# HuajianUP/Photo-SLAM

Hardware: AMD Instinct MI355X
Metric: train iters/s (render + L1/SSIM loss + backward + Adam), 2M Gaussians @1080p (higher is better)
Workload: dtype f32; 1 GPU; C3: Replica room0 @1080p shape; gaussians=2000000, width=1920, height=1080, sh_degree=3, parallelism=single GPU, raster_only=False, densify_interval=0, cull_empty_tiles=False, binning=depth-first, sh_adam_fused_into_backward=True, sh_adam_lazy_window=32, scene_index_order=random, geometry_adam_fused_into_backward=True, gaussians_after=2000000

## Files before the change

photo-slam_amd/csrc/preprocess.hip:

```cpp
#include "state.h"
#include "wave64.h"
#include "kernels.h"
#include "shrows.h"

namespace gsr {


__device__ __forceinline__ int f2i(float f)
{
	if (f != f) return 0;
	if (f >= 2147483648.0f) return 2147483647;
	if (f <= -2147483648.0f) return (-2147483647 - 1);
	return (int)f;
}

__device__ __forceinline__ float ndc2pix(float v, int S) { return (float)(((v + 1.0) * S - 1.0) * 0.5); }

#ifndef GSR_FWD_STAGE_ROWS
#define GSR_FWD_STAGE_ROWS STAGE_ROWS
#endif
constexpr int FWD_ROWS = GSR_FWD_STAGE_ROWS;

template <bool AA>
__global__ void __launch_bounds__(PRE_THREADS)
preprocess_fwd_kernel(const PreprocessParams p, GeometryState g)
{
	__shared__ float4 s_rows[PRE_THREADS / 64][FWD_ROWS][ROW_F4_PAD];
	__shared__ uint32_t s_list[PRE_THREADS / 64][64];
	__shared__ uint32_t s_lag[PRE_THREADS / 64][64];

	const int idx = (int)(blockIdx.x * blockDim.x + threadIdx.x);
	for (int t = idx; t < p.tiles; t += (int)(gridDim.x * blockDim.x)) p.ranges[t] = make_uint2(0u, 0u);
	for (int t = idx; t < LONG_LISTS * LONG_COUNT_STRIDE; t += (int)(gridDim.x * blockDim.x)) g.long_counts[t] = 0u;
	const int w = wave_id();
	const size_t wave_first = (size_t)(blockIdx.x * blockDim.x) + (size_t)w * 64;
	const bool in_range = idx < p.P;
	const int row_step = (p.lazy.row_step != nullptr && in_range) ? p.lazy.row_step[idx] : 0;
	uint32_t my_tiles = 0;
	int radius_i = 0;
	uint32_t depth_key = DEPTH_KEY_CULLED;
	float px = 0.f, py = 0.f, pz = 0.f;
	float pix = 0.f, piy = 0.f, conx = 0.f, cony = 0.f, conz = 0.f;
	uint32_t rect_lo = 0, rect_hi = 0;
	float aa_h = 1.0f;

	if (in_range) {
		do {
			px = p.means3D[3 * idx];
			py = p.means3D[3 * idx + 1];
			pz = p.means3D[3 * idx + 2];
			const float* V = p.view;
			const float* Pm = p.proj;
			const float vz = V[2] * px + V[6] * py + V[10] * pz + V[14];
			if (vz <= 0.2f) break;
			const float hx = Pm[0] * px + Pm[4] * py + Pm[8] * pz + Pm[12];
			const float hy = Pm[1] * px + Pm[5] * py + Pm[9] * pz + Pm[13];
			const float hw = Pm[3] * px + Pm[7] * py + Pm[11] * pz + Pm[15];
			const float p_w = 1.0f / (hw + 0.0000001f);
			const float projx = hx * p_w, projy = hy * p_w;

			float c3[6];
			if (p.cov3D_precomp != nullptr) {
#pragma unroll
				for (int i = 0; i < 6; i++) c3[i] = p.cov3D_precomp[6 * (size_t)idx + i];
			} else {
				compute_cov3D(p.scales, p.rotations, (size_t)idx, p.scale_modifier, p.raw_params, c3);
			}

			float tx = V[0] * px + V[4] * py + V[8] * pz + V[12];
			float ty = V[1] * px + V[5] * py + V[9] * pz + V[13];
			const float tz = vz;
			const float limx = 1.3f * p.tan_fovx, limy = 1.3f * p.tan_fovy;
			const float txtz = tx / tz, tytz = ty / tz;
			tx = fminf(limx, fmaxf(-limx, txtz)) * tz;
// ... 24 lines not shown
			const float lambda2 = mid - sqrtf(fmaxf(0.1f, mid * mid - det));
			const float my_radius = ceilf(3.f * sqrtf(fmaxf(lambda1, lambda2)));
			pix = ndc2pix(projx, p.W);
			piy = ndc2pix(projy, p.H);
			const int mr = f2i(my_radius);
			const int rminx = min(p.grid_x, max(0, f2i((pix - mr) / TILE)));
			const int rminy = min(p.grid_y, max(0, f2i((piy - mr) / TILE)));
			const int rmaxx = min(p.grid_x, max(0, f2i((pix + mr + TILE - 1) / TILE)));
			const int rmaxy = min(p.grid_y, max(0, f2i((piy + mr + TILE - 1) / TILE)));
			const uint32_t tiles = (uint32_t)(rmaxy - rminy) * (uint32_t)(rmaxx - rminx);
			if (tiles == 0) break;
			if (p.cov3D_precomp == nullptr && (p.raw_params & GSR_STORE_COV3D)) {
#pragma unroll
				for (int i = 0; i < 6; i++) g.cov3D[6 * (size_t)idx + i] = c3[i];
			}
			depth_key = __float_as_uint(vz);
			radius_i = mr;
			my_tiles = tiles;
			rect_lo = (uint32_t)rminx | ((uint32_t)rminy << 16);
			rect_hi = (uint32_t)rmaxx | ((uint32_t)rmaxy << 16);
		} while (0);
	}
	const bool vis = my_tiles != 0;

	float cr = 0.f, cg = 0.f, cb = 0.f;
	uint8_t clamp_bits = 0;
	if (p.colors_precomp == nullptr) {
		const int ncoef = (p.D + 1) * (p.D + 1);
		const bool rows_ok = (p.M * 3 == ROW_F4 * 4) && ((reinterpret_cast<uintptr_t>(p.shs) & 15) == 0);
		float rgb[3] = {0.f, 0.f, 0.f};
		auto direction = [&]() {
			const float dx = px - p.campos[0], dy = py - p.campos[1], dz = pz - p.campos[2];
			const float len = sqrtf(dx * dx + dy * dy + dz * dz);
			return sh_dir(dx / len, dy / len, dz / len);
		};
		if (rows_ok) {
			const unsigned long long vmask = wave_ballot(vis);
			const int nvis = __popcll(vmask);
			const int rank = __popcll(vmask & lanemask_lt());
			int lag = 0;
			if (p.lazy.row_step != nullptr && vis) {
				lag = p.lazy.step - 1 - row_step;
				lag = lag < 0 ? 0 : (lag >= p.lazy.window ? p.lazy.window - 1 : lag);
			}
			const bool lagging = wave_ballot(lag > 0) != 0;
			if (vis) {
				s_list[w][rank] = (uint32_t)lane_id();
				s_lag[w][rank] = (uint32_t)lag;
			}
			wave_fence();
			const int nf4 = lagging ? ROW_F4 : (3 * ncoef + 3) >> 2;
			for (int r0 = 0; r0 < nvis; r0 += FWD_ROWS) {
				const int count = (nvis - r0) < FWD_ROWS ? (nvis - r0) : FWD_ROWS;
				wave_load_listed_rows(reinterpret_cast<const float4*>(p.shs), wave_first, nf4, r0, count, s_rows[w], s_list[w]);
				if (lagging) {
					if (p.forward_only) wave_lazy_peek_listed(p.lazy, wave_first, r0, count, s_rows[w], s_list[w], s_lag[w]);
					else wave_lazy_catch_up_listed(p.lazy, wave_first, r0, count, s_rows[w], s_list[w], s_lag[w]);
				}
				if (vis && rank >= r0 && rank < r0 + count) sh_row_to_rgb(s_rows[w][rank - r0], ncoef, direction(), rgb);
				wave_fence();
			}
			if (lag > 0 && !p.forward_only) p.lazy.row_step[idx] = p.lazy.step - 1;
		} else if (vis) {
			const float* sh = p.shs + (size_t)idx * p.M * 3;
			const ShDir d = direction();
#pragma unroll
			for (int k = 0; k < 16; k++) {
				if (k < ncoef) {
#pragma unroll
					for (int ch = 0; ch < 3; ch++) {
						const float t = sh_basis(k, d) * sh[3 * k + ch];
						rgb[ch] = (k == 0) ? t : rgb[ch] + t;
					}
				}
			}
		}
		if (vis) {
			cr = rgb[0] + 0.5f;
			cg = rgb[1] + 0.5f;
			cb = rgb[2] + 0.5f;
			clamp_bits = (uint8_t)((cr < 0 ? 1 : 0) | (cg < 0 ? 2 : 0) | (cb < 0 ? 4 : 0));
			cr = fmaxf(cr, 0.0f);
			cg = fmaxf(cg, 0.0f);
			cb = fmaxf(cb, 0.0f);
		}
	} else if (vis) {
		cr = p.colors_precomp[3 * (size_t)idx];
		cg = p.colors_precomp[3 * (size_t)idx + 1];
		cb = p.colors_precomp[3 * (size_t)idx + 2];
	}

	if (in_range) {
		if (vis) {
			g.rec[3 * (size_t)idx + 0] = make_float4(pix, piy, conx, cony);
			float opac = p.opacities[idx];
			if (p.raw_params & GSR_RAW_OPACITY) opac = 1.0f / (1.0f + expf(-opac));
			if constexpr (AA) opac = opac * aa_h;
			g.rec[3 * (size_t)idx + 1] = make_float4(conz, opac, cr, cg);
			g.rec[3 * (size_t)idx + 2] = make_float4(cb, __uint_as_float(rect_lo), __uint_as_float(rect_hi), 0.f);
			if (!p.forward_only) g.clamped[idx] = clamp_bits;
			reinterpret_cast<uint2*>(g.rect)[idx] = make_uint2(rect_lo, rect_hi);
		}
		g.depth_key[idx] = depth_key;
		g.tiles_touched[idx] = my_tiles;
		g.radii[idx] = radius_i;
		if (p.radii_out) p.radii_out[idx] = radius_i;
	}
// ... 33 lines not shown
```

photo-slam_amd/csrc/preprocess_bwd.hip:

```cpp
#include "state.h"
#include "wave64.h"
#include <stdlib.h>
#include "kernels.h"
#include "shrows.h"
#include "partials.h"

namespace gsr {


constexpr int PRB_THREADS = 128;
constexpr int SHB_THREADS = 64;

template <int N>
__device__ __forceinline__ void geom_adam_row(const GeomAdamTensor& t, size_t idx, const float (&g)[N])
{
#pragma unroll
	for (int k = 0; k < N; k++) {
		const size_t i = (size_t)N * idx + k;
		const float m = t.s.b1 * t.exp_avg[i] + t.s.omb1 * g[k];
		const float v = t.s.b2 * t.exp_avg_sq[i] + t.s.omb2 * g[k] * g[k];
		t.exp_avg[i] = m;
		t.exp_avg_sq[i] = v;
		t.param[i] -= t.s.step_size * adam_ratio(m, v, t.s.inv_sqrt_bc2, t.s.eps);
	}
}
__device__ __forceinline__ void geom_adam_row4(const GeomAdamTensor& t, size_t idx, const float4& g4)
{
	float4 pv = reinterpret_cast<const float4*>(t.param)[idx];
	float4 mv = reinterpret_cast<const float4*>(t.exp_avg)[idx];
	float4 vv = reinterpret_cast<const float4*>(t.exp_avg_sq)[idx];
	float* pp = &pv.x; float* mp = &mv.x; float* vp = &vv.x;
	const float g[4] = {g4.x, g4.y, g4.z, g4.w};
#pragma unroll
	for (int k = 0; k < 4; k++) {
		mp[k] = t.s.b1 * mp[k] + t.s.omb1 * g[k];
		vp[k] = t.s.b2 * vp[k] + t.s.omb2 * g[k] * g[k];
		pp[k] -= t.s.step_size * adam_ratio(mp[k], vp[k], t.s.inv_sqrt_bc2, t.s.eps);
	}
	reinterpret_cast<float4*>(t.param)[idx] = pv;
	reinterpret_cast<float4*>(t.exp_avg)[idx] = mv;
	reinterpret_cast<float4*>(t.exp_avg_sq)[idx] = vv;
}

template <int DEG, int MODE, bool POSE = false>
#ifndef GSR_SHB_WAVES_LO
#define GSR_SHB_WAVES_LO 6
#endif
__global__ void __launch_bounds__(SHB_THREADS) GSR_WAVES_PER_EU(GSR_SHB_WAVES_LO, 8)
sh_bwd_rows_kernel(const PreprocessBwdParams p)
{
	__shared__ float4 s_rows[SHB_THREADS / 64][STAGE_ROWS][ROW_F4_PAD];
	__shared__ uint32_t s_list[SHB_THREADS / 64][STAGE_ROWS];
	__shared__ float s_aux[SHB_THREADS / 64][MODE == 2 ? STAGE_ROWS : 1][AUX_PITCH];
	const int idx = (int)(blockIdx.x * blockDim.x + threadIdx.x);
	const int w = wave_id(), l = lane_id();
	const size_t wave_first = (size_t)(blockIdx.x * blockDim.x) + (size_t)w * 64;
	if (p.touched_clear)
		for (uint32_t o = 16u * (uint32_t)idx; o < p.touched_clear_bytes; o += 16u * (uint32_t)(gridDim.x * blockDim.x))
			*reinterpret_cast<uint4*>(p.touched_clear + o) = make_uint4(0u, 0u, 0u, 0u);
	const bool in_range = idx < p.P;
	const bool vis = in_range && (p.radii[idx] > 0);
	constexpr int ncoef = (DEG + 1) * (DEG + 1);
	constexpr bool FACTORED = MODE == 1;
	float dRGB[3] = {0.f, 0.f, 0.f};
	float ddx[3] = {0.f, 0.f, 0.f}, ddy[3] = {0.f, 0.f, 0.f}, ddz[3] = {0.f, 0.f, 0.f};
	float ox = 0.f, oy = 0.f, oz = 1.f;
	if (vis) {
		ox = p.means3D[3 * (size_t)idx] - p.campos[0];
		oy = p.means3D[3 * (size_t)idx + 1] - p.campos[1];
		oz = p.means3D[3 * (size_t)idx + 2] - p.campos[2];
		if (FACTORED) {
			dRGB[0] = p.dL_dcolor_view[3 * (size_t)idx + 0];
			dRGB[1] = p.dL_dcolor_view[3 * (size_t)idx + 1];
			dRGB[2] = p.dL_dcolor_view[3 * (size_t)idx + 2];
		} else {
			const uint8_t cl = p.clamped[idx];
			dRGB[0] = p.dL_dcolor[3 * (size_t)idx + 0] * ((cl & 1) ? 0.f : 1.f);
			dRGB[1] = p.dL_dcolor[3 * (size_t)idx + 1] * ((cl & 2) ? 0.f : 1.f);
			dRGB[2] = p.dL_dcolor[3 * (size_t)idx + 2] * ((cl & 4) ? 0.f : 1.f);
		}
	}
	{
		{
			const int nf4 = MODE == 2 ? ROW_F4 : (3 * ncoef + 3) >> 2;
#pragma unroll 1
			for (int h = 0; h < 64 / STAGE_ROWS; h++) {
				const size_t half_first = wave_first + (size_t)(h * STAGE_ROWS);
				const long long left = (long long)p.P - (long long)half_first;
				if (left <= 0) break;
				const bool mine = (l / STAGE_ROWS) == h;
				const unsigned long long m = wave_ballot(vis && mine);
				if (vis && mine) s_list[w][__popcll(m & lanemask_lt())] = (uint32_t)(l % STAGE_ROWS);
				wave_fence();
				wave_load_listed_rows<true>(reinterpret_cast<const float4*>(p.shs), half_first, nf4, 0, __popcll(m), s_rows[w], s_list[w]);
				if (mine && in_range) {
					float4* row = s_rows[w][l % STAGE_ROWS];
					if (vis) {
						float ux = ox, uy = oy, uz = oz;
						GSR_OPAQUE_F32(ux);
						GSR_OPAQUE_F32(uy);
						GSR_OPAQUE_F32(uz);
						const float len = sqrtf(ux * ux + uy * uy + uz * uz);
						const ShDir d = sh_dir(ux / len, uy / len, uz / len);
						sh_row_backward<MODE == 0>(row, ncoef, d, dRGB, ddx, ddy, ddz);
						if (MODE == 2) {
							float* ax = s_aux[w][l % STAGE_ROWS];
#pragma unroll
							for (int k = 0; k < 16; k++) ax[k] = k < ncoef ? sh_basis(k, d) : 0.f;
							ax[16] = dRGB[0];
							ax[17] = dRGB[1];
							ax[18] = dRGB[2];
						}
					} else if (MODE == 0) {
#pragma unroll
						for (int i = 0; i < ROW_F4; i++) row[i] = make_float4(0.f, 0.f, 0.f, 0.f);
					}
				}
				if (MODE == 0) {
					wave_store_rows(reinterpret_cast<float4*>(p.dL_dsh), half_first, (int)(left > STAGE_ROWS ? STAGE_ROWS : left), s_rows[w]);
				} else if (MODE == 2) {
					const RowAdam ra = {p.adam_param, p.adam_exp_avg, p.adam_exp_avg_sq, p.adam};
					const uint32_t lit = (uint32_t)(m >> (h * STAGE_ROWS));
					const uint32_t rows = p.adam_skip_culled ? lit : 0xFFFFFFFFu;
					wave_adam_rows_rank1(ra, half_first, (int)(left > STAGE_ROWS ? STAGE_ROWS : left), s_rows[w], s_aux[w], rows, lit);
				} else {
					wave_fence();
				}
			}
		}
	}
	if (MODE == 2 && vis && p.lazy_row_step) p.lazy_row_step[idx] = p.lazy_step;
	float gm[3] = {0.f, 0.f, 0.f};
	float gc[3] = {0.f, 0.f, 0.f};
	if (vis) {
		const float dLx = ddx[0] * dRGB[0] + ddx[1] * dRGB[1] + ddx[2] * dRGB[2];
		const float dLy = ddy[0] * dRGB[0] + ddy[1] * dRGB[1] + ddy[2] * dRGB[2];
		const float dLz = ddz[0] * dRGB[0] + ddz[1] * dRGB[1] + ddz[2] * dRGB[2];
		const float sum2 = ox * ox + oy * oy + oz * oz;
		const float invsum32 = 1.0f / sqrtf(sum2 * sum2 * sum2);
		gm[0] = p.dL_dmean3D[3 * (size_t)idx + 0] + ((+sum2 - ox * ox) * dLx - oy * ox * dLy - oz * ox * dLz) * invsum32;
		gm[1] = p.dL_dmean3D[3 * (size_t)idx + 1] + (-ox * oy * dLx + (sum2 - oy * oy) * dLy - oz * oy * dLz) * invsum32;
		gm[2] = p.dL_dmean3D[3 * (size_t)idx + 2] + (-ox * oz * dLx - oy * oz * dLy + (sum2 - oz * oz) * dLz) * invsum32;
		if constexpr (POSE) {
			gc[0] = -(((+sum2 - ox * ox) * dLx - oy * ox * dLy - oz * ox * dLz) * invsum32);
			gc[1] = -((-ox * oy * dLx + (sum2 - oy * oy) * dLy - oz * oy * dLz) * invsum32);
			gc[2] = -((-ox * oz * dLx - oy * oz * dLy + (sum2 - oz * oz) * dLz) * invsum32);
		}
		if (!p.geom.on) {
			p.dL_dmean3D[3 * (size_t)idx + 0] = gm[0];
			p.dL_dmean3D[3 * (size_t)idx + 1] = gm[1];
			p.dL_dmean3D[3 * (size_t)idx + 2] = gm[2];
		}
	}
	if (p.geom.on && in_range) geom_adam_row<3>(p.geom.xyz, (size_t)idx, gm);
	if constexpr (POSE) {
		float* slab_b = p.pose_scratch + (size_t)POSE_VP * (((size_t)p.P + PRB_THREADS - 1) / PRB_THREADS);
#pragma unroll
		for (int k = 0; k < 3; k++) {
			const float c = wave_sum_f32_lane63(gc[k]);
			if (l == 63) slab_b[(size_t)k * gridDim.x + blockIdx.x] = c;
		}
	}
}

__device__ __forceinline__ void pack_view_row(const PreprocessBwdParams& p, int idx, bool vis, unsigned long long seen_mask, float v0, float v1,
                                              float v2)
{
	const size_t groups = ((size_t)p.P + 63) >> 6;
	const size_t prefix_words = (groups + 3) & ~(size_t)3, mask_words = (2 * groups + 3) & ~(size_t)3;
	uint32_t* msg = p.packed_msg;
	const size_t group = (size_t)idx >> 6;
	const uint32_t first = msg[PACK_HEADER + group];
	if (vis) {
		const uint32_t rank = first + (uint32_t)__popcll(seen_mask & lanemask_lt());
		if (rank < (uint32_t)p.packed_capacity) {
			float* rows = reinterpret_cast<float*>(msg + PACK_HEADER + prefix_words + mask_words);
			rows[3 * (size_t)rank] = v0;
// ... 316 lines not shown
		float4 q = reinterpret_cast<const float4*>(p.rotations)[idx];
		float qn = 1.0f;
		if (p.raw_params & GSR_RAW_ROTATION) {
			qn = fmaxf(sqrtf(q.x * q.x + q.y * q.y + q.z * q.z + q.w * q.w), 1e-12f);
			q.x = q.x / qn;
			q.y = q.y / qn;
			q.z = q.z / qn;
			q.w = q.w / qn;
		}
		const float r = q.x, x = q.y, y = q.z, z = q.w;
		float sx = p.scales[3 * (size_t)idx], sy = p.scales[3 * (size_t)idx + 1], sz = p.scales[3 * (size_t)idx + 2];
		if (p.raw_params & GSR_RAW_SCALING) {
			sx = expf(sx);
			sy = expf(sy);
			sz = expf(sz);
		}
		const float s0 = p.scale_modifier * sx, s1 = p.scale_modifier * sy, s2 = p.scale_modifier * sz;
		const float R00 = 1.f - 2.f * (y * y + z * z), R01 = 2.f * (x * y - r * z), R02 = 2.f * (x * z + r * y);
		const float R10 = 2.f * (x * y + r * z), R11 = 1.f - 2.f * (x * x + z * z), R12 = 2.f * (y * z - r * x);
		const float R20 = 2.f * (x * z - r * y), R21 = 2.f * (y * z + r * x), R22 = 1.f - 2.f * (x * x + y * y);
		const float N00 = 2.0f * (s0 * R00), N01 = 2.0f * (s1 * R01), N02 = 2.0f * (s2 * R02);
		const float N10 = 2.0f * (s0 * R10), N11 = 2.0f * (s1 * R11), N12 = 2.0f * (s2 * R12);
		const float N20 = 2.0f * (s0 * R20), N21 = 2.0f * (s1 * R21), N22 = 2.0f * (s2 * R22);
		const float S00 = dcov[0], S01 = 0.5f * dcov[1], S02 = 0.5f * dcov[2];
		const float S11 = dcov[3], S12 = 0.5f * dcov[4], S22 = dcov[5];
		const float S10 = S01, S20 = S02, S21 = S12;
#define DM(c_, r_) (N0##r_ * S##c_##0 + N1##r_ * S##c_##1 + N2##r_ * S##c_##2)
		float D00 = DM(0, 0), D01 = DM(1, 0), D02 = DM(2, 0);
		float D10 = DM(0, 1), D11 = DM(1, 1), D12 = DM(2, 1);
		float D20 = DM(0, 2), D21 = DM(1, 2), D22 = DM(2, 2);
#undef DM
		const float ds0 = R00 * D00 + R10 * D01 + R20 * D02, ds1 = R01 * D10 + R11 * D11 + R21 * D12,
		            ds2 = R02 * D20 + R12 * D21 + R22 * D22;
		const bool raw_s = (p.raw_params & GSR_RAW_SCALING) != 0;
		g_scale[0] = raw_s ? ds0 * sx : ds0;
		g_scale[1] = raw_s ? ds1 * sy : ds1;
		g_scale[2] = raw_s ? ds2 * sz : ds2;
		D00 *= s0; D01 *= s0; D02 *= s0;
		D10 *= s1; D11 *= s1; D12 *= s1;
		D20 *= s2; D21 *= s2; D22 *= s2;
		dq.x = 2 * z * (D01 - D10) + 2 * y * (D20 - D02) + 2 * x * (D12 - D21);
		dq.y = 2 * y * (D10 + D01) + 2 * z * (D20 + D02) + 2 * r * (D12 - D21) - 4 * x * (D22 + D11);
		dq.z = 2 * x * (D10 + D01) + 2 * r * (D20 - D02) + 2 * z * (D12 + D21) - 4 * y * (D22 + D00);
		dq.w = 2 * r * (D01 - D10) + 2 * x * (D20 + D02) + 2 * y * (D12 + D21) - 4 * z * (D11 + D00);
		if (p.raw_params & GSR_RAW_ROTATION) {
			const float qg = r * dq.x + x * dq.y + y * dq.z + z * dq.w;
			dq.x = (dq.x - r * qg) / qn;
			dq.y = (dq.y - x * qg) / qn;
			dq.z = (dq.z - y * qg) / qn;
			dq.w = (dq.w - z * qg) / qn;
		}
	}
	if (in_range && p.geom.on) {
		geom_adam_row<3>(p.geom.scaling, (size_t)idx, g_scale);
		geom_adam_row4(p.geom.rotation, (size_t)idx, dq);
	} else if (in_range && p.dL_dscale) {
		p.dL_dscale[3 * (size_t)idx + 0] = g_scale[0];
		p.dL_dscale[3 * (size_t)idx + 1] = g_scale[1];
		p.dL_dscale[3 * (size_t)idx + 2] = g_scale[2];
		reinterpret_cast<float4*>(p.dL_drot)[idx] = dq;
	}
	if constexpr (POSE) {
		const int l = lane_id(), w = wave_id();
		float packed[3];
		wave_reduce24_swap_f32(pose_v, packed);
		if ((l & 7) == 0) {
#pragma unroll
			for (int j = 0; j < 3; j++) s_pose[w][8 * j + wave_swap9_component(l)] = packed[j];
		}
		if (!rows_ok) {
#pragma unroll
			for (int k = 0; k < 3; k++) {
				const float c = wave_sum_f32_lane63(pose_c[k]);
				if (l == 63) s_pose[w][POSE_VP + k] = c;
			}
		}
		__syncthreads();
		const int t = (int)threadIdx.x;
		if (t < (rows_ok ? POSE_VP : POSE_VP + 3)) {
			float sum = s_pose[0][t];
#pragma unroll
			for (int k = 1; k < PRB_THREADS / 64; k++) sum += s_pose[k][t];
			p.pose_scratch[(size_t)t * gridDim.x + blockIdx.x] = sum;
		}
	}
}

__device__ __forceinline__ void sh_adam_culled_item(long long t, const int* __restrict__ radii, const RowAdam& a)
{
	const long long row = t / ROW_F4;
	if (radii[row] > 0) return;
	const int col = (int)(t - row * ROW_F4);
	const size_t i = (size_t)t;
	float4 pv = load_stream_f4(reinterpret_cast<const float4*>(a.param) + i);
	float4 mv = load_stream_f4(reinterpret_cast<const float4*>(a.exp_avg) + i);
	float4 vv = load_stream_f4(reinterpret_cast<const float4*>(a.exp_avg_sq) + i);
	float* pp = &pv.x; float* mp = &mv.x; float* vp = &vv.x;
	const float ss_first = col == 0 ? a.s.step_size : a.s.step_size_tail;
#pragma unroll
	for (int e = 0; e < 4; e++) {
		const float ss = e < 3 ? ss_first : a.s.step_size_tail;
		const float g = 0.f;
		mp[e] = a.s.b1 * mp[e] + a.s.omb1 * g;
		vp[e] = a.s.b2 * vp[e] + a.s.omb2 * g * g;
		pp[e] -= ss * adam_ratio(mp[e], vp[e], a.s.inv_sqrt_bc2, a.s.eps);
	}
	store_stream_f4(reinterpret_cast<float4*>(a.param) + i, pv);
	store_stream_f4(reinterpret_cast<float4*>(a.exp_avg) + i, mv);
// ... 497 lines not shown
```

photo-slam_amd/csrc/shrows.h:

```cpp
#pragma once
#include "state.h"
#include "wave64.h"
#include "kernels.h"

namespace gsr {

constexpr int ROW_F4 = 12;
constexpr int ROW_F4_PAD = 13;
#ifndef GSR_STAGE_ROWS
#define GSR_STAGE_ROWS 32
#endif
constexpr int STAGE_ROWS = GSR_STAGE_ROWS;

template <bool BY_SOURCE = false>
__device__ __forceinline__ void wave_load_listed_rows(const float4* __restrict__ gbase, size_t first_row, int nf4, int list_first,
                                                      int count, float4 (*s_rows)[ROW_F4_PAD], const uint32_t* s_list)
{
	const int l = lane_id();
	const int slot = l >> 4, col = l & 15;
	for (int j0 = 0; j0 < count; j0 += 4) {
		const int j = j0 + slot;
		if (col < nf4 && j < count) {
			const uint32_t src = s_list[list_first + j];
			s_rows[BY_SOURCE ? (int)src : j][col] = load_stream_f4(gbase + (first_row + src) * ROW_F4 + col);
		}
	}
	wave_fence();
}

__device__ __forceinline__ void wave_store_rows(float4* __restrict__ gbase, size_t first_row, int nrows,
                                                float4 (*s_rows)[ROW_F4_PAD])
{
	const int l = lane_id();
	const int slot = l >> 4, col = l & 15;
	wave_fence();
	float4* dst = gbase + (first_row + slot) * ROW_F4 + col;
	const float4* src = &s_rows[slot][col];
#pragma unroll
	for (int k = 0; k < STAGE_ROWS / 4; k++) {
		if (col < ROW_F4 && 4 * k + slot < nrows) dst[4 * k * ROW_F4] = src[4 * k * ROW_F4_PAD];
	}
	wave_fence();
}

__device__ __forceinline__ float adam_ratio(float m, float v, float c2, float eps)
{
#ifdef GSR_EMU
	return m * (1.0f / (sqrtf(v) * c2 + eps));
#else
	return m * __builtin_amdgcn_rcpf(__builtin_amdgcn_sqrtf(v) * c2 + eps);
#endif
}

struct RowAdam {
	float* param;
	float* exp_avg;
	float* exp_avg_sq;
	AdamScalars s;
};
__device__ __forceinline__ void lazy_zero_grad_steps(const LazyAdamTable& t, int k_hi, int k_lo, int col, float4& pv, float4& mv,
                                                     float4& vv);
template <bool CATCH_UP = false>
__device__ __forceinline__ void wave_adam_rows(const RowAdam& a, size_t first_row, int nrows, float4 (*s_rows)[ROW_F4_PAD],
                                               uint32_t row_mask = 0xFFFFFFFFu, const LazyAdamTable* t = nullptr,
                                               const uint32_t* s_lag = nullptr)
{
	const int l = lane_id();
	const int slot = l >> 4, col = l & 15;
	wave_fence();
	const size_t base = (first_row + slot) * ROW_F4 + col;
	const float ss_first = col == 0 ? a.s.step_size : a.s.step_size_tail;
#ifndef GSR_ADAM_UNROLL
#define GSR_ADAM_UNROLL 2
#endif
#pragma unroll GSR_ADAM_UNROLL
	for (int k = 0; k < STAGE_ROWS / 4; k++) {
		if (col < ROW_F4 && 4 * k + slot < nrows && ((row_mask >> (4 * k + slot)) & 1u)) {
			const size_t i = base + (size_t)(4 * k * ROW_F4);
			const float4 gv = s_rows[4 * k + slot][col];
			float4 pv = load_stream_f4(reinterpret_cast<const float4*>(a.param) + i);
			float4 mv = load_stream_f4(reinterpret_cast<const float4*>(a.exp_avg) + i);
			float4 vv = load_stream_f4(reinterpret_cast<const float4*>(a.exp_avg_sq) + i);
			if (CATCH_UP) {
				const int lag = (int)s_lag[4 * k + slot];
				if (lag > 0) lazy_zero_grad_steps(*t, lag, 1, col, pv, mv, vv);
			}
			float* pp = &pv.x; const float* gp = &gv.x; float* mp = &mv.x; float* vp = &vv.x;
#pragma unroll
			for (int e = 0; e < 4; e++) {
				const float ss = e < 3 ? ss_first : a.s.step_size_tail;
				mp[e] = a.s.b1 * mp[e] + a.s.omb1 * gp[e];
				vp[e] = a.s.b2 * vp[e] + a.s.omb2 * gp[e] * gp[e];
				pp[e] -= ss * adam_ratio(mp[e], vp[e], a.s.inv_sqrt_bc2, a.s.eps);
			}
			store_stream_f4(reinterpret_cast<float4*>(a.param) + i, pv);
			store_stream_f4(reinterpret_cast<float4*>(a.exp_avg) + i, mv);
			store_stream_f4(reinterpret_cast<float4*>(a.exp_avg_sq) + i, vv);
		}
	}
	wave_fence();
}

constexpr int AUX_PITCH = 21;
__device__ __forceinline__ void wave_adam_rows_rank1(const RowAdam& a, size_t first_row, int nrows, float4 (*s_rows)[ROW_F4_PAD],
                                                     const float (*s_aux)[AUX_PITCH], uint32_t row_mask, uint32_t vis_mask)
{
	const int l = lane_id();
	const int slot = l >> 4, col = l & 15;
	wave_fence();
	const size_t base = (first_row + slot) * ROW_F4 + col;
	const float ss_first = col == 0 ? a.s.step_size : a.s.step_size_tail;
	int kc[4], cc[4];
#pragma unroll
	for (int c = 0; c < 4; c++) {
		const int e = (4 * col + c) % (4 * ROW_F4);
		kc[c] = e / 3;
		cc[c] = 16 + e - 3 * kc[c];
	}
#pragma unroll GSR_ADAM_UNROLL
	for (int k = 0; k < STAGE_ROWS / 4; k++) {
		const int r = 4 * k + slot;
		if (col < ROW_F4 && r < nrows && ((row_mask >> r) & 1u)) {
			const size_t i = base + (size_t)(4 * k * ROW_F4);
			float4 mv = load_stream_f4(reinterpret_cast<const float4*>(a.exp_avg) + i);
			float4 vv = load_stream_f4(reinterpret_cast<const float4*>(a.exp_avg_sq) + i);
			float4 pv, gv;
			if ((vis_mask >> r) & 1u) {
				pv = s_rows[r][col];
				const float* ax = s_aux[r];
				gv = make_float4(ax[kc[0]] * ax[cc[0]], ax[kc[1]] * ax[cc[1]], ax[kc[2]] * ax[cc[2]], ax[kc[3]] * ax[cc[3]]);
			} else {
				pv = load_stream_f4(reinterpret_cast<const float4*>(a.param) + i);
				gv = make_float4(0.f, 0.f, 0.f, 0.f);
			}
			float* pp = &pv.x; const float* gp = &gv.x; float* mp = &mv.x; float* vp = &vv.x;
#pragma unroll
			for (int e = 0; e < 4; e++) {
				const float ss = e < 3 ? ss_first : a.s.step_size_tail;
				mp[e] = a.s.b1 * mp[e] + a.s.omb1 * gp[e];
				vp[e] = a.s.b2 * vp[e] + a.s.omb2 * gp[e] * gp[e];
				pp[e] -= ss * adam_ratio(mp[e], vp[e], a.s.inv_sqrt_bc2, a.s.eps);
			}
			store_stream_f4(reinterpret_cast<float4*>(a.param) + i, pv);
			store_stream_f4(reinterpret_cast<float4*>(a.exp_avg) + i, mv);
			store_stream_f4(reinterpret_cast<float4*>(a.exp_avg_sq) + i, vv);
		}
	}
	wave_fence();
}


__device__ __forceinline__ void lazy_zero_grad_steps(const LazyAdamTable& t, int k_hi, int k_lo, int col, float4& pv, float4& mv,
                                                     float4& vv)
{
	float* pp = &pv.x; float* mp = &mv.x; float* vp = &vv.x;
	for (int k = k_hi; k >= k_lo; k--) {
		const float tail = t.step_size_tail[k];
		const float ss_first = col == 0 ? t.step_size[k] : tail;
		const float c2 = t.inv_sqrt_bc2[k];
#pragma unroll
		for (int e = 0; e < 4; e++) {
			const float ss = e < 3 ? ss_first : tail;
			const float g = 0.f;
			mp[e] = t.b1 * mp[e] + t.omb1 * g;
			vp[e] = t.b2 * vp[e] + t.omb2 * g * g;
			pp[e] -= ss * adam_ratio(mp[e], vp[e], c2, t.eps);
		}
	}
}

__device__ __forceinline__ void wave_lazy_catch_up_listed(const LazyAdam& a, size_t first_row, int list_first, int count,
                                                          float4 (*s_rows)[ROW_F4_PAD], const uint32_t* s_list, const uint32_t* s_lag)
{
	const int l = lane_id();
	const int slot = l >> 4, col = l & 15;
	wave_fence();
	for (int j0 = 0; j0 < count; j0 += 4) {
		const int j = j0 + slot;
		if (col < ROW_F4 && j < count) {
			const int lag = (int)s_lag[list_first + j];
			if (lag > 0) {
				const size_t i = (first_row + s_list[list_first + j]) * ROW_F4 + col;
				float4 pv = s_rows[j][col];
				float4 mv = load_stream_f4(reinterpret_cast<const float4*>(a.exp_avg) + i);
				float4 vv = load_stream_f4(reinterpret_cast<const float4*>(a.exp_avg_sq) + i);
				lazy_zero_grad_steps(a.t, lag, 1, col, pv, mv, vv);
				store_stream_f4(reinterpret_cast<float4*>(a.param) + i, pv);
				store_stream_f4(reinterpret_cast<float4*>(a.exp_avg) + i, mv);
				store_stream_f4(reinterpret_cast<float4*>(a.exp_avg_sq) + i, vv);
				s_rows[j][col] = pv;
			}
		}
	}
	wave_fence();
}

__device__ __forceinline__ void wave_lazy_peek_listed(const LazyAdam& a, size_t first_row, int list_first, int count,
                                                      float4 (*s_rows)[ROW_F4_PAD], const uint32_t* s_list, const uint32_t* s_lag)
// ... 135 lines not shown
```

photo-slam_amd/csrc/wave64.h:

```cpp
#pragma once
#include "rt.h"

namespace gsr {

#ifdef GSR_EMU
using ::hipemu::wave_ballot;
using ::hipemu::wave_fence;
using ::hipemu::wave_incl_scan_u32;
using ::hipemu::wave_max_u32;
using ::hipemu::wave_reduce9_f32;
using ::hipemu::wave_shfl_u32;
using ::hipemu::wave_sum_u32;
using ::hipemu::wave_uniform_u64;
using ::hipemu::wave_uniform_u32;
using ::hipemu::wave_readlane_f32;
using ::hipemu::wave_readlane_u32;
using ::hipemu::wave_writelane_f32;
using ::hipemu::wave_reduce9_swap_f32;
using ::hipemu::wave_swap9_component;
using ::hipemu::mask_select_f32;
using ::hipemu::mask_select_u32;
using ::hipemu::mask_select0_f32;
#define GSR_OPAQUE_F32(x) asm volatile("" : "+x"(x))
static inline float wave_xor_add_f32(float v, int mask)
{
	uint32_t b;
	memcpy(&b, &v, 4);
	b = wave_shfl_u32(b, ::hipemu::lane() ^ mask);
	float o;
	memcpy(&o, &b, 4);
	return v + o;
}
static inline float wave_row_sum16_f32(float v)
{
	v = wave_xor_add_f32(v, 1);
	v = wave_xor_add_f32(v, 2);
	v = wave_xor_add_f32(v, 7);
	return wave_xor_add_f32(v, 15);
}
static inline float wave_sum_f32_lane63(float v)
{
	v = wave_row_sum16_f32(v);
	float r[4];
	for (int k = 0; k < 4; k++) r[k] = wave_readlane_f32(v, 16 * k + 15);
	return (r[3] + r[2]) + (r[1] + r[0]);
}
static inline void wave_reduce10_swap_f32(const float (&v)[10], float& packed, float& ninth_row, float& tenth_row)
{
	float t[9];
	for (int c = 0; c < 9; c++) t[c] = v[c];
	uint32_t b8, b9;
	memcpy(&b8, &v[8], 4);
	memcpy(&b9, &v[9], 4);
	const uint64_t* s = ::hipemu::wave_exchange((uint64_t)b8 | ((uint64_t)b9 << 32));
	float r8 = 0.f, r9 = 0.f;
	for (int i = 0; i < 16; i++) {
		const uint64_t w = s[(::hipemu::lane() & ~15) + i];
		const uint32_t lo = (uint32_t)w, hi = (uint32_t)(w >> 32);
		float f8, f9;
		memcpy(&f8, &lo, 4);
		memcpy(&f9, &hi, 4);
		r8 += f8;
		r9 += f9;
	}
	::hipemu::wave_sync();
	wave_reduce9_f32(t);
	packed = t[wave_swap9_component(::hipemu::lane())];
	ninth_row = r8;
	tenth_row = r9;
}
static inline float4 load_stream_f4(const float4* p) { return *p; }
static inline void store_stream_f4(float4* p, const float4 v) { *p = v; }
#define GSR_SCHED_BARRIER() ((void)0)
#else

__device__ __forceinline__ float wave_readlane_f32(float v, int lane)
{
	return __builtin_bit_cast(float, __builtin_amdgcn_readlane(__builtin_bit_cast(int, v), lane));
}
__device__ __forceinline__ uint32_t wave_readlane_u32(uint32_t v, int lane) { return (uint32_t)__builtin_amdgcn_readlane((int)v, lane); }
__device__ __forceinline__ float wave_writelane_f32(float old, float uniform_value, int lane)
{
	return ((int)(threadIdx.x & 63u) == lane) ? uniform_value : old;
}

__device__ __forceinline__ uint32_t wave_uniform_u32(uint32_t v) { return (uint32_t)__builtin_amdgcn_readfirstlane((int)v); }
__device__ __forceinline__ unsigned long long wave_uniform_u64(unsigned long long v)
{
	const uint32_t lo = (uint32_t)__builtin_amdgcn_readfirstlane((int)(uint32_t)v);
	const uint32_t hi = (uint32_t)__builtin_amdgcn_readfirstlane((int)(uint32_t)(v >> 32));
	return ((unsigned long long)hi << 32) | lo;
}

__device__ __forceinline__ unsigned long long wave_ballot(bool pred) { return __builtin_amdgcn_ballot_w64(pred); }

__device__ __forceinline__ float mask_select_f32(unsigned long long mask, float if_set, float if_clear)
{
	float r;
	asm("v_cndmask_b32 %0, %1, %2, %3" : "=v"(r) : "v"(if_clear), "v"(if_set), "s"(mask));
	return r;
}
__device__ __forceinline__ uint32_t mask_select_u32(unsigned long long mask, uint32_t if_set, uint32_t if_clear)
{
	uint32_t r;
	asm("v_cndmask_b32 %0, %1, %2, %3" : "=v"(r) : "v"(if_clear), "v"(if_set), "s"(mask));
	return r;
}
__device__ __forceinline__ float mask_select0_f32(unsigned long long mask, float if_set)
{
	float r;
	asm("v_cndmask_b32 %0, 0, %1, %2" : "=v"(r) : "v"(if_set), "s"(mask));
	return r;
}

__device__ __forceinline__ float4 load_stream_f4(const float4* p)
{
	typedef float v4f __attribute__((ext_vector_type(4)));
	const v4f t = __builtin_nontemporal_load(reinterpret_cast<const v4f*>(p));
	return make_float4(t.x, t.y, t.z, t.w);
}

__device__ __forceinline__ void store_stream_f4(float4* p, const float4 v)
{
	typedef float v4f __attribute__((ext_vector_type(4)));
	v4f t = {v.x, v.y, v.z, v.w};
	__builtin_nontemporal_store(t, reinterpret_cast<v4f*>(p));
}

#define GSR_OPAQUE_F32(x) asm volatile("" : "+v"(x))
#define GSR_SCHED_BARRIER()                \
	do {                                   \
		asm volatile("" ::: "memory");     \
		__builtin_amdgcn_sched_barrier(0); \
	} while (0)

__device__ __forceinline__ void wave_fence()
{
	__builtin_amdgcn_fence(__ATOMIC_RELEASE, "wavefront");
	__builtin_amdgcn_wave_barrier();
	__builtin_amdgcn_fence(__ATOMIC_ACQUIRE, "wavefront");
}

__device__ __forceinline__ uint32_t wave_shfl_u32(uint32_t v, int src_lane) { return (uint32_t)__shfl((int)v, src_lane, 64); }

template <int CTRL, int ROW_MASK = 0xf, int BANK_MASK = 0xf, bool BOUND_CTRL = true>
__device__ __forceinline__ float dpp_f32(float old_v, float v)
{
	return __builtin_bit_cast(float, __builtin_amdgcn_update_dpp(__builtin_bit_cast(int, old_v), __builtin_bit_cast(int, v),
	                                                              CTRL, ROW_MASK, BANK_MASK, BOUND_CTRL));
}
template <int CTRL, int ROW_MASK = 0xf, int BANK_MASK = 0xf, bool BOUND_CTRL = true>
__device__ __forceinline__ uint32_t dpp_u32(uint32_t old_v, uint32_t v)
{
	return (uint32_t)__builtin_amdgcn_update_dpp((int)old_v, (int)v, CTRL, ROW_MASK, BANK_MASK, BOUND_CTRL);
}

constexpr int DPP_QUAD_PERM_1032 = 0xB1;
constexpr int DPP_QUAD_PERM_2301 = 0x4E;
constexpr int DPP_ROW_SHR1 = 0x111;
constexpr int DPP_ROW_SHR2 = 0x112;
constexpr int DPP_ROW_SHR4 = 0x114;
constexpr int DPP_ROW_SHR8 = 0x118;
constexpr int DPP_ROW_MIRROR = 0x140;
constexpr int DPP_ROW_HALF_MIRROR = 0x141;
constexpr int DPP_ROW_BCAST15 = 0x142;
constexpr int DPP_ROW_BCAST31 = 0x143;

__device__ __forceinline__ float wave_sum_f32_lane63(float v)
{
	v += dpp_f32<DPP_QUAD_PERM_1032>(0.f, v);
	v += dpp_f32<DPP_QUAD_PERM_2301>(0.f, v);
	v += dpp_f32<DPP_ROW_HALF_MIRROR>(0.f, v);
	v += dpp_f32<DPP_ROW_MIRROR>(0.f, v);
	v += dpp_f32<DPP_ROW_BCAST15, 0xa>(0.f, v);
	v += dpp_f32<DPP_ROW_BCAST31, 0xc>(0.f, v);
	return v;
}

__device__ __forceinline__ float wave_row_sum16_f32(float v)
{
	v += dpp_f32<DPP_QUAD_PERM_1032>(0.f, v);
	v += dpp_f32<DPP_QUAD_PERM_2301>(0.f, v);
	v += dpp_f32<DPP_ROW_HALF_MIRROR>(0.f, v);
	v += dpp_f32<DPP_ROW_MIRROR>(0.f, v);
	return v;
}

// ... 143 lines not shown
```

Measured before the change: 656.1 iters/s.

## Batch SH row and Adam loads ahead of use to raise memory-level parallelism

Restructures the listed-row SH loader, the rank-1 SH Adam update and the geometry Adam so that several groups of global loads are issued into registers before one explicit vmcnt wait, and only then consumed and stored. The rank-1 Adam also gains a compacted path that walks only the visible-row list when culled rows are skipped. The aim is to hide global memory latency in the bandwidth-bound preprocess and SH backward kernels by keeping more loads in flight. In exchange it raises register pressure, which may lower occupancy, and relies on a hand-coded waitcnt immediate.

```diff
diff --git a/photo-slam_amd/csrc/preprocess.hip b/photo-slam_amd/csrc/preprocess.hip
--- a/photo-slam_amd/csrc/preprocess.hip
+++ b/photo-slam_amd/csrc/preprocess.hip
@@ -20,6 +20,10 @@
 #define GSR_FWD_STAGE_ROWS STAGE_ROWS
 #endif
 constexpr int FWD_ROWS = GSR_FWD_STAGE_ROWS;
+#ifndef GSR_FWD_TRIP_GROUPS
+#define GSR_FWD_TRIP_GROUPS 4
+#endif
+constexpr int FWD_TRIP_GROUPS = GSR_FWD_TRIP_GROUPS;
 
 template <bool AA>
 __global__ void __launch_bounds__(PRE_THREADS)
@@ -150,7 +154,7 @@
 			const int nf4 = lagging ? ROW_F4 : (3 * ncoef + 3) >> 2;
 			for (int r0 = 0; r0 < nvis; r0 += FWD_ROWS) {
 				const int count = (nvis - r0) < FWD_ROWS ? (nvis - r0) : FWD_ROWS;
-				wave_load_listed_rows(reinterpret_cast<const float4*>(p.shs), wave_first, nf4, r0, count, s_rows[w], s_list[w]);
+				wave_load_listed_rows<false, FWD_TRIP_GROUPS>(reinterpret_cast<const float4*>(p.shs), wave_first, nf4, r0, count, s_rows[w], s_list[w]);
 				if (lagging) {
 					if (p.forward_only) wave_lazy_peek_listed(p.lazy, wave_first, r0, count, s_rows[w], s_list[w], s_lag[w]);
 					else wave_lazy_catch_up_listed(p.lazy, wave_first, r0, count, s_rows[w], s_list[w], s_lag[w]);
diff --git a/photo-slam_amd/csrc/preprocess_bwd.hip b/photo-slam_amd/csrc/preprocess_bwd.hip
--- a/photo-slam_amd/csrc/preprocess_bwd.hip
+++ b/photo-slam_amd/csrc/preprocess_bwd.hip
@@ -12,24 +12,56 @@
 constexpr int SHB_THREADS = 64;
 
 template <int N>
-__device__ __forceinline__ void geom_adam_row(const GeomAdamTensor& t, size_t idx, const float (&g)[N])
+struct GeomAdamRegs {
+	float m[N], v[N], w[N];
+};
+template <int N>
+__device__ __forceinline__ void geom_adam_load(const GeomAdamTensor& t, size_t idx, GeomAdamRegs<N>& r)
 {
 #pragma unroll
 	for (int k = 0; k < N; k++) {
 		const size_t i = (size_t)N * idx + k;
-		const float m = t.s.b1 * t.exp_avg[i] + t.s.omb1 * g[k];
-		const float v = t.s.b2 * t.exp_avg_sq[i] + t.s.omb2 * g[k] * g[k];
-		t.exp_avg[i] = m;
-		t.exp_avg_sq[i] = v;
-		t.param[i] -= t.s.step_size * adam_ratio(m, v, t.s.inv_sqrt_bc2, t.s.eps);
-	}
-}
-__device__ __forceinline__ void geom_adam_row4(const GeomAdamTensor& t, size_t idx, const float4& g4)
-{
-	float4 pv = reinterpret_cast<const float4*>(t.param)[idx];
-	float4 mv = reinterpret_cast<const float4*>(t.exp_avg)[idx];
-	float4 vv = reinterpret_cast<const float4*>(t.exp_avg_sq)[idx];
-	float* pp = &pv.x; float* mp = &mv.x; float* vp = &vv.x;
+		r.m[k] = t.exp_avg[i];
+		r.v[k] = t.exp_avg_sq[i];
+		r.w[k] = t.param[i];
+	}
+}
+template <int N>
+__device__ __forceinline__ void geom_adam_finish(const GeomAdamTensor& t, size_t idx, const float (&g)[N], GeomAdamRegs<N>& r)
+{
+#pragma unroll
+	for (int k = 0; k < N; k++) {
+		r.m[k] = t.s.b1 * r.m[k] + t.s.omb1 * g[k];
+		r.v[k] = t.s.b2 * r.v[k] + t.s.omb2 * g[k] * g[k];
+		r.w[k] -= t.s.step_size * adam_ratio(r.m[k], r.v[k], t.s.inv_sqrt_bc2, t.s.eps);
+	}
+#pragma unroll
+	for (int k = 0; k < N; k++) {
+		const size_t i = (size_t)N * idx + k;
+		t.exp_avg[i] = r.m[k];
+		t.exp_avg_sq[i] = r.v[k];
+		t.param[i] = r.w[k];
+	}
+}
+template <int N>
+__device__ __forceinline__ void geom_adam_row(const GeomAdamTensor& t, size_t idx, const float (&g)[N])
+{
+	GeomAdamRegs<N> r;
+	geom_adam_load<N>(t, idx, r);
+	geom_adam_finish<N>(t, idx, g, r);
+}
+struct GeomAdamRegs4 {
+	float4 p, m, v;
+};
+__device__ __forceinline__ void geom_adam_load4(const GeomAdamTensor& t, size_t idx, GeomAdamRegs4& r)
+{
+	r.p = reinterpret_cast<const float4*>(t.param)[idx];
+	r.m = reinterpret_cast<const float4*>(t.exp_avg)[idx];
+	r.v = reinterpret_cast<const float4*>(t.exp_avg_sq)[idx];
+}
+__device__ __forceinline__ void geom_adam_finish4(const GeomAdamTensor& t, size_t idx, const float4& g4, GeomAdamRegs4& r)
+{
+	float* pp = &r.p.x; float* mp = &r.m.x; float* vp = &r.v.x;
 	const float g[4] = {g4.x, g4.y, g4.z, g4.w};
 #pragma unroll
 	for (int k = 0; k < 4; k++) {
@@ -37,12 +69,15 @@
 		vp[k] = t.s.b2 * vp[k] + t.s.omb2 * g[k] * g[k];
 		pp[k] -= t.s.step_size * adam_ratio(mp[k], vp[k], t.s.inv_sqrt_bc2, t.s.eps);
 	}
-	reinterpret_cast<float4*>(t.param)[idx] = pv;
-	reinterpret_cast<float4*>(t.exp_avg)[idx] = mv;
-	reinterpret_cast<float4*>(t.exp_avg_sq)[idx] = vv;
+	reinterpret_cast<float4*>(t.param)[idx] = r.p;
+	reinterpret_cast<float4*>(t.exp_avg)[idx] = r.m;
+	reinterpret_cast<float4*>(t.exp_avg_sq)[idx] = r.v;
 }
 
 template <int DEG, int MODE, bool POSE = false>
+#ifndef GSR_SHB_SMALL_TRIP
+#define GSR_SHB_SMALL_TRIP 4
+#endif
 #ifndef GSR_SHB_WAVES_LO
 #define GSR_SHB_WAVES_LO 6
 #endif
@@ -62,6 +97,7 @@
 	const bool vis = in_range && (p.radii[idx] > 0);
 	constexpr int ncoef = (DEG + 1) * (DEG + 1);
 	constexpr bool FACTORED = MODE == 1;
+	constexpr int SHB_TRIP_GROUPS = MODE == 2 ? STAGE_ROWS / 4 : (STAGE_ROWS / 4 > GSR_SHB_SMALL_TRIP ? GSR_SHB_SMALL_TRIP : STAGE_ROWS / 4);
 	float dRGB[3] = {0.f, 0.f, 0.f};
 	float ddx[3] = {0.f, 0.f, 0.f}, ddy[3] = {0.f, 0.f, 0.f}, ddz[3] = {0.f, 0.f, 0.f};
 	float ox = 0.f, oy = 0.f, oz = 1.f;
@@ -92,7 +128,7 @@
 				const unsigned long long m = wave_ballot(vis && mine);
 				if (vis && mine) s_list[w][__popcll(m & lanemask_lt())] = (uint32_t)(l % STAGE_ROWS);
 				wave_fence();
-				wave_load_listed_rows<true>(reinterpret_cast<const float4*>(p.shs), half_first, nf4, 0, __popcll(m), s_rows[w], s_list[w]);
+				wave_load_listed_rows<true, SHB_TRIP_GROUPS>(reinterpret_cast<const float4*>(p.shs), half_first, nf4, 0, __popcll(m), s_rows[w], s_list[w]);
 				if (mine && in_range) {
 					float4* row = s_rows[w][l % STAGE_ROWS];
 					if (vis) {
@@ -122,7 +158,8 @@
 					const RowAdam ra = {p.adam_param, p.adam_exp_avg, p.adam_exp_avg_sq, p.adam};
 					const uint32_t lit = (uint32_t)(m >> (h * STAGE_ROWS));
 					const uint32_t rows = p.adam_skip_culled ? lit : 0xFFFFFFFFu;
-					wave_adam_rows_rank1(ra, half_first, (int)(left > STAGE_ROWS ? STAGE_ROWS : left), s_rows[w], s_aux[w], rows, lit);
+					wave_adam_rows_rank1(ra, half_first, (int)(left > STAGE_ROWS ? STAGE_ROWS : left), s_rows[w], s_aux[w], rows, lit,
+					                     p.adam_skip_culled ? s_list[w] : nullptr, __popcll(m));
 				} else {
 					wave_fence();
 				}
@@ -545,8 +582,12 @@
 		}
 	}
 	if (in_range && p.geom.on) {
-		geom_adam_row<3>(p.geom.scaling, (size_t)idx, g_scale);
-		geom_adam_row4(p.geom.rotation, (size_t)idx, dq);
+		GeomAdamRegs<3> rs;
+		GeomAdamRegs4 rq;
+		geom_adam_load<3>(p.geom.scaling, (size_t)idx, rs);
+		geom_adam_load4(p.geom.rotation, (size_t)idx, rq);
+		geom_adam_finish<3>(p.geom.scaling, (size_t)idx, g_scale, rs);
+		geom_adam_finish4(p.geom.rotation, (size_t)idx, dq, rq);
 	} else if (in_range && p.dL_dscale) {
 		p.dL_dscale[3 * (size_t)idx + 0] = g_scale[0];
 		p.dL_dscale[3 * (size_t)idx + 1] = g_scale[1];
diff --git a/photo-slam_amd/csrc/shrows.h b/photo-slam_amd/csrc/shrows.h
--- a/photo-slam_amd/csrc/shrows.h
+++ b/photo-slam_amd/csrc/shrows.h
@@ -12,17 +12,28 @@
 #endif
 constexpr int STAGE_ROWS = GSR_STAGE_ROWS;
 
-template <bool BY_SOURCE = false>
+template <bool BY_SOURCE = false, int TRIP_GROUPS = STAGE_ROWS / 4>
 __device__ __forceinline__ void wave_load_listed_rows(const float4* __restrict__ gbase, size_t first_row, int nf4, int list_first,
                                                       int count, float4 (*s_rows)[ROW_F4_PAD], const uint32_t* s_list)
 {
 	const int l = lane_id();
 	const int slot = l >> 4, col = l & 15;
-	for (int j0 = 0; j0 < count; j0 += 4) {
-		const int j = j0 + slot;
-		if (col < nf4 && j < count) {
-			const uint32_t src = s_list[list_first + j];
-			s_rows[BY_SOURCE ? (int)src : j][col] = load_stream_f4(gbase + (first_row + src) * ROW_F4 + col);
+#pragma unroll 1
+	for (int j0 = 0; j0 < count; j0 += 4 * TRIP_GROUPS) {
+		float4 v[TRIP_GROUPS];
+#pragma unroll
+		for (int k = 0; k < TRIP_GROUPS; k++) {
+			const int j = j0 + 4 * k + slot;
+			if (col < nf4 && j < count) {
+				const uint32_t src = s_list[list_first + j];
+				v[k] = load_stream_f4(gbase + (first_row + src) * ROW_F4 + col);
+			}
+		}
+		GSR_WAIT_LOADS();
+#pragma unroll
+		for (int k = 0; k < TRIP_GROUPS; k++) {
+			const int j = j0 + 4 * k + slot;
+			if (col < nf4 && j < count) s_rows[BY_SOURCE ? (int)s_list[list_first + j] : j][col] = v[k];
 		}
 	}
 	wave_fence();
@@ -102,13 +113,31 @@
 }
 
 constexpr int AUX_PITCH = 21;
+__device__ __forceinline__ void rank1_vector_step(const RowAdam& a, float ss_first, float4& pv, const float4& gv, float4& mv, float4& vv)
+{
+	float* pp = &pv.x; const float* gp = &gv.x; float* mp = &mv.x; float* vp = &vv.x;
+#pragma unroll
+	for (int e = 0; e < 4; e++) {
+		const float ss = e < 3 ? ss_first : a.s.step_size_tail;
+		mp[e] = a.s.b1 * mp[e] + a.s.omb1 * gp[e];
+		vp[e] = a.s.b2 * vp[e] + a.s.omb2 * gp[e] * gp[e];
+		pp[e] -= ss * adam_ratio(mp[e], vp[e], a.s.inv_sqrt_bc2, a.s.eps);
+	}
+}
+#ifndef GSR_RANK1_LIST_GROUPS
+#define GSR_RANK1_LIST_GROUPS 4
+#endif
+constexpr int RANK1_LIST_GROUPS = GSR_RANK1_LIST_GROUPS;
+#ifndef GSR_RANK1_MASKED_GROUPS
+#define GSR_RANK1_MASKED_GROUPS 2
+#endif
 __device__ __forceinline__ void wave_adam_rows_rank1(const RowAdam& a, size_t first_row, int nrows, float4 (*s_rows)[ROW_F4_PAD],
-                                                     const float (*s_aux)[AUX_PITCH], uint32_t row_mask, uint32_t vis_mask)
-{
-	const int l = lane_id();
-	const int slot = l >> 4, col = l & 15;
-	wave_fence();
-	const size_t base = (first_row + slot) * ROW_F4 + col;
+                                                     const float (*s_aux)[AUX_PITCH], uint32_t row_mask, uint32_t vis_mask,
+                                                     const uint32_t* s_list = nullptr, int count = 0)
+{
+	const int l = lane_id();
+	const int slot = l >> 4, col = l & 15;
+	wave_fence();
 	const float ss_first = col == 0 ? a.s.step_size : a.s.step_size_tail;
 	int kc[4], cc[4];
 #pragma unroll
@@ -117,33 +146,75 @@
 		kc[c] = e / 3;
 		cc[c] = 16 + e - 3 * kc[c];
 	}
-#pragma unroll GSR_ADAM_UNROLL
-	for (int k = 0; k < STAGE_ROWS / 4; k++) {
-		const int r = 4 * k + slot;
-		if (col < ROW_F4 && r < nrows && ((row_mask >> r) & 1u)) {
-			const size_t i = base + (size_t)(4 * k * ROW_F4);
-			float4 mv = load_stream_f4(reinterpret_cast<const float4*>(a.exp_avg) + i);
-			float4 vv = load_stream_f4(reinterpret_cast<const float4*>(a.exp_avg_sq) + i);
-			float4 pv, gv;
-			if ((vis_mask >> r) & 1u) {
-				pv = s_rows[r][col];
-				const float* ax = s_aux[r];
-				gv = make_float4(ax[kc[0]] * ax[cc[0]], ax[kc[1]] * ax[cc[1]], ax[kc[2]] * ax[cc[2]], ax[kc[3]] * ax[cc[3]]);
-			} else {
-				pv = load_stream_f4(reinterpret_cast<const float4*>(a.param) + i);
-				gv = make_float4(0.f, 0.f, 0.f, 0.f);
-			}
-			float* pp = &pv.x; const float* gp = &gv.x; float* mp = &mv.x; float* vp = &vv.x;
-#pragma unroll
-			for (int e = 0; e < 4; e++) {
-				const float ss = e < 3 ? ss_first : a.s.step_size_tail;
-				mp[e] = a.s.b1 * mp[e] + a.s.omb1 * gp[e];
-				vp[e] = a.s.b2 * vp[e] + a.s.omb2 * gp[e] * gp[e];
-				pp[e] -= ss * adam_ratio(mp[e], vp[e], a.s.inv_sqrt_bc2, a.s.eps);
-			}
-			store_stream_f4(reinterpret_cast<float4*>(a.param) + i, pv);
-			store_stream_f4(reinterpret_cast<float4*>(a.exp_avg) + i, mv);
-			store_stream_f4(reinterpret_cast<float4*>(a.exp_avg_sq) + i, vv);
+	if (s_list != nullptr) {
+#pragma unroll 1
+		for (int j0 = 0; j0 < count; j0 += 4 * RANK1_LIST_GROUPS) {
+			float4 mv[RANK1_LIST_GROUPS], vv[RANK1_LIST_GROUPS];
+			int r[RANK1_LIST_GROUPS];
+#pragma unroll
+			for (int b = 0; b < RANK1_LIST_GROUPS; b++) {
+				const int j = j0 + 4 * b + slot;
+				if (col < ROW_F4 && j < count) {
+					r[b] = (int)s_list[j];
+					const size_t i = (first_row + (size_t)r[b]) * ROW_F4 + col;
+					mv[b] = load_stream_f4(reinterpret_cast<const float4*>(a.exp_avg) + i);
+					vv[b] = load_stream_f4(reinterpret_cast<const float4*>(a.exp_avg_sq) + i);
+				}
+			}
+			GSR_WAIT_LOADS();
+#pragma unroll
+			for (int b = 0; b < RANK1_LIST_GROUPS; b++) {
+				const int j = j0 + 4 * b + slot;
+				if (col < ROW_F4 && j < count) {
+					const size_t i = (first_row + (size_t)r[b]) * ROW_F4 + col;
+					float4 pv = s_rows[r[b]][col];
+					const float* ax = s_aux[r[b]];
+					const float4 gv = make_float4(ax[kc[0]] * ax[cc[0]], ax[kc[1]] * ax[cc[1]], ax[kc[2]] * ax[cc[2]], ax[kc[3]] * ax[cc[3]]);
+					rank1_vector_step(a, ss_first, pv, gv, mv[b], vv[b]);
+					store_stream_f4(reinterpret_cast<float4*>(a.param) + i, pv);
+					store_stream_f4(reinterpret_cast<float4*>(a.exp_avg) + i, mv[b]);
+					store_stream_f4(reinterpret_cast<float4*>(a.exp_avg_sq) + i, vv[b]);
+				}
+			}
+		}
+		wave_fence();
+		return;
+	}
+	const size_t base = (first_row + slot) * ROW_F4 + col;
+	constexpr int ADAM_BATCH = GSR_RANK1_MASKED_GROUPS;
+	static_assert((STAGE_ROWS / 4) % ADAM_BATCH == 0, "a trip takes ADAM_BATCH whole row groups");
+#pragma unroll 1
+	for (int k0 = 0; k0 < STAGE_ROWS / 4; k0 += ADAM_BATCH) {
+		float4 pv[ADAM_BATCH], mv[ADAM_BATCH], vv[ADAM_BATCH];
+#pragma unroll
+		for (int b = 0; b < ADAM_BATCH; b++) {
+			const int r = 4 * (k0 + b) + slot;
+			if (col < ROW_F4 && r < nrows && ((row_mask >> r) & 1u)) {
+				const size_t i = base + (size_t)(4 * (k0 + b) * ROW_F4);
+				mv[b] = load_stream_f4(reinterpret_cast<const float4*>(a.exp_avg) + i);
+				vv[b] = load_stream_f4(reinterpret_cast<const float4*>(a.exp_avg_sq) + i);
+				if (!((vis_mask >> r) & 1u)) pv[b] = load_stream_f4(reinterpret_cast<const float4*>(a.param) + i);
+			}
+		}
+		GSR_WAIT_LOADS();
+#pragma unroll
+		for (int b = 0; b < ADAM_BATCH; b++) {
+			const int r = 4 * (k0 + b) + slot;
+			if (col < ROW_F4 && r < nrows && ((row_mask >> r) & 1u)) {
+				const size_t i = base + (size_t)(4 * (k0 + b) * ROW_F4);
+				float4 gv;
+				if ((vis_mask >> r) & 1u) {
+					pv[b] = s_rows[r][col];
+					const float* ax = s_aux[r];
+					gv = make_float4(ax[kc[0]] * ax[cc[0]], ax[kc[1]] * ax[cc[1]], ax[kc[2]] * ax[cc[2]], ax[kc[3]] * ax[cc[3]]);
+				} else {
+					gv = make_float4(0.f, 0.f, 0.f, 0.f);
+				}
+				rank1_vector_step(a, ss_first, pv[b], gv, mv[b], vv[b]);
+				store_stream_f4(reinterpret_cast<float4*>(a.param) + i, pv[b]);
+				store_stream_f4(reinterpret_cast<float4*>(a.exp_avg) + i, mv[b]);
+				store_stream_f4(reinterpret_cast<float4*>(a.exp_avg_sq) + i, vv[b]);
+			}
 		}
 	}
 	wave_fence();
diff --git a/photo-slam_amd/csrc/wave64.h b/photo-slam_amd/csrc/wave64.h
--- a/photo-slam_amd/csrc/wave64.h
+++ b/photo-slam_amd/csrc/wave64.h
@@ -72,6 +72,7 @@
 static inline float4 load_stream_f4(const float4* p) { return *p; }
 static inline void store_stream_f4(float4* p, const float4 v) { *p = v; }
 #define GSR_SCHED_BARRIER() ((void)0)
+#define GSR_WAIT_LOADS() ((void)0)
 #else
 
 __device__ __forceinline__ float wave_readlane_f32(float v, int lane)
@@ -133,6 +134,8 @@
 		asm volatile("" ::: "memory");     \
 		__builtin_amdgcn_sched_barrier(0); \
 	} while (0)
+
+#define GSR_WAIT_LOADS() __builtin_amdgcn_s_waitcnt(0x0F70)
 
 __device__ __forceinline__ void wave_fence()
 {
```

New measurement: 679.4 iters/s (median of 6 runs). +3.5%, better.
